# compix/Monte-Carlo-Raytracer

Measured on AMD Instinct MI355X. Metric: Mpaths/sec + achieved HBM GB/s, San-Miguel 1920x1080 at 1/2/4/8 MI355X, higher is better.
Workload: dtype f32; 1 GPU; san_miguel_proxy 1920x1080, unidirectional PT, maxDepth 2, random sampler, 1 spp per step, box-filter accumulate; width=1920, height=1080, triangles=9984786, max_depth=2, global_batch=1, bvh=RadeonRays-identical SAH, device build, parallelism=tile-split 8-row bands x 1 + 1 RCCL band gather, frames_per_launch=32, max_frames_per_call=32

## Files before the change

### include/mcrt_capi.h

```cpp
#ifndef MCRT_CAPI_H
#define MCRT_CAPI_H

#include <stddef.h>
#include <stdint.h>

#ifdef __cplusplus
extern "C" {
#endif

#define MCRT_API __attribute__((visibility("default")))

typedef int mcrt_status;
#define MCRT_OK                   0
#define MCRT_ERROR_INVALID_ARG    1
#define MCRT_ERROR_OUT_OF_MEMORY  2
#define MCRT_ERROR_DEVICE         3
#define MCRT_ERROR_NOT_READY      4
#define MCRT_ERROR_NO_DEVICE      5

typedef struct __attribute__((aligned(16))) { float x, y, z, w; } mcrt_float4;
typedef mcrt_float4 mcrt_float3;
typedef struct __attribute__((aligned(8))) { float x, y; } mcrt_float2;
typedef struct __attribute__((aligned(16))) { mcrt_float4 m0, m1, m2, m3; } mcrt_mat4;

// ... 164 lines not shown
MCRT_API mcrt_status mcrt_ctx_gather_chase_compact(mcrt_ctx ctx, uint64_t records, double leaf_frac, int steps,
                                                   int iters, double* gsteps);

MCRT_API mcrt_status mcrt_scene_create(mcrt_ctx ctx, const mcrt_scene_desc* desc, mcrt_scene* out);
MCRT_API mcrt_status mcrt_scene_destroy(mcrt_scene scene);
MCRT_API mcrt_status mcrt_scene_update_lights(mcrt_scene scene, const mcrt_light* lights, uint32_t n);
MCRT_API mcrt_status mcrt_scene_update_materials(mcrt_scene scene, const mcrt_material* m, uint32_t n);
MCRT_API mcrt_status mcrt_scene_update_shapes(mcrt_scene scene, const mcrt_shape* s, uint32_t n);
MCRT_API mcrt_status mcrt_scene_update_vertices(mcrt_scene scene, uint32_t first, uint32_t count,
                                                const mcrt_float4* positions, const mcrt_float4* normals);
MCRT_API mcrt_status mcrt_scene_update_vertices_device(mcrt_scene scene, uint32_t first, uint32_t count,
                                                       const void* d_positions, const void* d_normals);
MCRT_API mcrt_status mcrt_accel_build(mcrt_scene scene, const mcrt_accel_opts* opts);
MCRT_API mcrt_status mcrt_accel_update_transforms(mcrt_scene scene, const mcrt_shape* shapes, uint32_t n,
                                                  const mcrt_mat4* world_to_local );
MCRT_API mcrt_status mcrt_accel_refit(mcrt_scene scene);
MCRT_API mcrt_status mcrt_accel_update_info(mcrt_scene scene, int32_t* path, double* ms);
MCRT_API mcrt_status mcrt_accel_info(mcrt_scene scene, uint64_t* num_nodes, uint64_t* device_bytes,
                                     double* build_ms, uint32_t* num_triangles);
MCRT_API mcrt_status mcrt_accel_layout(mcrt_scene scene, int32_t* two_level, uint32_t* num_meshes,
                                       uint32_t* num_instances, int32_t* depth);
MCRT_API mcrt_status mcrt_accel_read_records(mcrt_scene scene, float* out, uint64_t max_records,
                                             uint64_t* num_records);
typedef struct mcrt_obj_scene_s* mcrt_obj_scene;
#define MCRT_OBJ_MIPS            1
#define MCRT_OBJ_EMISSIVE_LIGHTS 2
MCRT_API mcrt_status mcrt_obj_load(const char* path, uint32_t flags, mcrt_obj_scene* out);
MCRT_API mcrt_status mcrt_obj_add_directional_light(mcrt_obj_scene s, const float dir[3], const float intensity[3]);
MCRT_API mcrt_status mcrt_obj_add_point_light(mcrt_obj_scene s, const float pos[3], const float intensity[3]);
MCRT_API mcrt_status mcrt_obj_scene_desc(mcrt_obj_scene s, mcrt_scene_desc* desc);
MCRT_API const char* mcrt_obj_warnings(mcrt_obj_scene s);
MCRT_API void mcrt_obj_free(mcrt_obj_scene s);

MCRT_API mcrt_status mcrt_accel_builder(mcrt_scene scene, int32_t* builder);
MCRT_API mcrt_status mcrt_accel_build_host_records(const mcrt_scene_desc* desc, const mcrt_accel_opts* opts,
                                                   float* out_records, uint64_t max_records,
                                                   uint64_t* num_records, int32_t* info);

MCRT_API mcrt_status mcrt_accel_refit_host_records(const mcrt_scene_desc* desc, const mcrt_accel_opts* opts,
                                                   const mcrt_shape* moved_shapes,
                                                   const mcrt_mat4* moved_world_to_local,
                                                   float* out_records, uint64_t max_records,
                                                   uint64_t* num_records, int32_t* info);

MCRT_API mcrt_status mcrt_trace_closest(mcrt_scene scene, const mcrt_ray* d_rays, int32_t n,
                                        mcrt_intersection* d_hits);
// ... 176 lines not shown
```

### monte-carlo-raytracer_amd/csrc/mcrt_accel.cpp

```cpp
#include <hip/hip_runtime.h>

#include <algorithm>
#include <cassert>
#include <chrono>
#include <cstdio>
#include <cstdlib>
#include <cstring>
#include <string>
#include <vector>

#include "mcrt_host.h"

using mcrt::fail, mcrt::env_int;
using Clock = std::chrono::steady_clock;

static double ms_since(Clock::time_point t0) {
    return std::chrono::duration<double, std::milli>(Clock::now() - t0).count();
}

bool mcrt::accel_ready(mcrt_scene s) { return (bool)s->accel.dNodes; }
const float4* mcrt::accel_nodes(mcrt_scene s) { return s->accel.dNodes.get(); }
int mcrt::accel_spill_cap(mcrt_scene s) { return s->accel.spillCap; }
const float* mcrt::accel_world_box(mcrt_scene s) { return s->accel.tree.box; }

// ... 95 lines not shown
    a.refitParent.reset();
    a.refitArrive.reset();
    a.refitQOff.reset();
    a.refitFlag.reset();
    a.tree = mcrt::TreeInfo();
    a.qRoot = 0;
    a.packets = false;
}

static mcrt_status finish(mcrt_scene s, bool boxFromRoot) {
    mcrt_ctx ctx = s->ctx;
    AccelState& a = s->accel;
    mcrt::TreeInfo& t = a.tree;
    a.packets = !t.twoLevel && 2 * t.depth <= MCRT_PK_STACK && t.numNodes < (1u << 26) &&
                env_int("MCRT_CAMERA_PACKETS", 1) != 0;
    if (!a.dScratch) HIPCHK(ctx, a.dScratch.alloc(256));
    HIPCHK(ctx, hipMemset(a.dScratch.get(), 0, 256 * sizeof(int)));
    if (!t.twoLevel) {
        mcrt::launch_leaf_parents(a.dNodes.get(), (uint32_t)t.numNodes, ctx->stream);
        HIPCHK(ctx, hipStreamSynchronize(ctx->stream));
    }
    if (!t.twoLevel && env_int("MCRT_QUANT_NODES", 1) != 0) {
        DevBuf<float4> q;
        const hipError_t e = mcrt::build_qnodes(a.dNodes.get(), (uint32_t)t.numNodes, q, ctx->stream);
        if (e == hipSuccess) {
            a.dQNodes = std::move(q);
        } else if (e != hipErrorNotSupported && e != hipErrorOutOfMemory) {
            return fail(ctx, MCRT_ERROR_DEVICE, std::string("compact records: ") + hipGetErrorString(e));
        } else {
            (void)hipGetLastError();
        }
    }
    apply_spill_cap(a);
    if (boxFromRoot) {
        float root[16];
        HIPCHK(ctx, hipMemcpy(root, a.dNodes.get(), sizeof(root), hipMemcpyDeviceToHost));
        mcrt::root_record_box(root, t.box);
    }
    a.qRoot = !t.twoLevel && t.numNodes == 1 ? 1u : 0u;
    return MCRT_OK;
}

static mcrt_status commit(mcrt_scene s, const mcrt_accel_opts* opts, DevBuf<float4>& nodes, const mcrt::TreeInfo& info,
                          mcrt::HostTree* host, Clock::time_point t0) {
    AccelState& a = s->accel;
    drop(a);
    a.dNodes = std::move(nodes);
// ... 157 lines not shown
    HIPCHK(ctx, hipStreamSynchronize(ctx->stream));
    HIPCHK(ctx, hipDeviceSynchronize());
    if (a.tree.twoLevel) {
        mcrt_accel_opts o = a.lastOpts;
        const mcrt_status st = mcrt_accel_build(s, a.haveOpts ? &o : nullptr);
        if (st != MCRT_OK) return st;
        a.updatePath = 3;
        a.updateMs = ms_since(t0);
        return MCRT_OK;
    }
    hipStream_t st = ctx->stream;
    const uint32_t n = (uint32_t)a.tree.numNodes;
    [[maybe_unused]] const int depth0 = a.tree.depth, cap0 = a.spillCap;
    [[maybe_unused]] const bool packets0 = a.packets;
    if (!a.refitParent) {
        DevBuf<int> parent, arrive, flag;
        DevBuf<uint32_t> qoff;
        HIPCHK(ctx, parent.alloc(n));
        HIPCHK(ctx, arrive.alloc(n));
        HIPCHK(ctx, flag.alloc(4));
        HIPCHK(ctx, mcrt::launch_refit_parents(a.dNodes.get(), n, parent.get(), st));
        if (a.dQNodes) {
            size_t total = 0;
            HIPCHK(ctx, mcrt::refit_qnode_offsets(a.dNodes.get(), n, qoff, &total, st));
            if (total != a.dQNodes.size()) return fail(ctx, MCRT_ERROR_DEVICE, "compact records: size changed without a build");
        }
        a.refitParent = std::move(parent);
        a.refitArrive = std::move(arrive);
        a.refitFlag = std::move(flag);
        a.refitQOff = std::move(qoff);
    }
    {
        Timed t(ctx, K_REFIT, nullptr, (int64_t)n);
        HIPCHK(ctx, mcrt::launch_refit(a.dNodes.get(), n, s->dShapes.get(), (uint32_t)s->shapes.size(), s->dIndices.get(),
                                       s->dPositions.get(), a.refitParent.get(), a.refitArrive.get(), st));
    }
    int unbounded = 0;
    if (a.dQNodes) {
        Timed t(ctx, K_REFIT_QNODES, nullptr, (int64_t)n);
        HIPCHK(ctx, mcrt::refit_qnodes(a.dNodes.get(), n, a.refitQOff.get(), a.dQNodes.get(), a.refitFlag.get(), st));
    }
    float root[16];
    if (a.dQNodes) HIPCHK(ctx, hipMemcpyAsync(&unbounded, a.refitFlag.get(), sizeof(int), hipMemcpyDeviceToHost, st));
    HIPCHK(ctx, hipMemcpyAsync(root, a.dNodes.get(), sizeof(root), hipMemcpyDeviceToHost, st));
    HIPCHK(ctx, hipStreamSynchronize(st));
    if (unbounded) {
        a.dQNodes.reset();
// ... 29 lines not shown
    if (!s) return fail(nullptr, MCRT_ERROR_INVALID_ARG, "scene is NULL");
    const AccelState& a = s->accel;
    if (!a.dNodes) return fail(s->ctx, MCRT_ERROR_NOT_READY, "mcrt_accel_build has not been called");
    if (two_level) *two_level = a.tree.twoLevel ? 1 : 0;
    if (num_meshes) *num_meshes = (uint32_t)a.tree.numMeshes;
    if (num_instances) *num_instances = (uint32_t)a.tree.numInstances;
    if (depth) *depth = a.tree.depth;
    return MCRT_OK;
}

MCRT_API mcrt_status mcrt_accel_read_records(mcrt_scene s, float* out, uint64_t max_records, uint64_t* num_records) {
    if (!s || !num_records) return fail(s ? s->ctx : nullptr, MCRT_ERROR_INVALID_ARG, "NULL argument");
    const AccelState& a = s->accel;
    if (!a.dNodes) return fail(s->ctx, MCRT_ERROR_INVALID_ARG, "scene has no acceleration structure");
    *num_records = a.tree.numNodes;
    if (!out) return MCRT_OK;
    mcrt_ctx ctx = s->ctx;
    hipSetDevice(ctx->device);
    HIPCHK(ctx, hipStreamSynchronize(ctx->stream));
    HIPCHK(ctx, hipMemcpy(out, a.dNodes.get(), 64 * std::min<uint64_t>(max_records, a.tree.numNodes), hipMemcpyDeviceToHost));
    return MCRT_OK;
}

MCRT_API mcrt_status mcrt_accel_builder(mcrt_scene s, int32_t* builder) {
    if (!s || !builder) return fail(s ? s->ctx : nullptr, MCRT_ERROR_INVALID_ARG, "NULL argument");
    *builder = s->accel.tree.builder;
    return MCRT_OK;
}

}
```

### monte-carlo-raytracer_amd/csrc/mcrt_host.h

```cpp
#pragma once
#include <climits>
#include <cstddef>
#include <string>
#include <vector>

#include "mcrt_devbuf.h"
#include "mcrt_internal.h"

using mcrt::DevBuf;

#define MCRT_ATROUS_MAX_LEVELS 8

enum KernelId {
    K_PRIMARY, K_SHADE0, K_SHADEN, K_SHADOW, K_EXTEND, K_ACCUM, K_TRACE_CLOSEST, K_TRACE_ANY,
    K_BDPT_START, K_BDPT_VERTEX, K_BDPT_CONNECT, K_BDPT_VIS, K_BDPT_GATHER, K_SHADOW_EXTEND,
    K_GUIDES, K_MOMENTS, K_ATROUS_PREP,
    K_ATROUS,
    K_TEMPORAL = K_ATROUS + MCRT_ATROUS_MAX_LEVELS, K_TEMPORAL_VAR, K_GUIDES_MOTION, K_TEMPORAL_MOTION,
    K_TILE_ERROR, K_TILE_LIST,
    K_REFIT, K_REFIT_QNODES,
    K_COUNT
};

struct mcrt_ctx_s {
// ... 2 lines not shown
    hipStream_t stream = nullptr;
    int numCUs = 256;
    bool profiling = false;
    bool countHints = false;
    int* dFlags = nullptr;
    std::string error;
    struct Pending {
        int kernel;
        hipEvent_t a, b;
        const int* countDev;
        const int* countDev2;
        int64_t items;
    };
    std::vector<Pending> pending;
    double totalMs[K_COUNT] = {};
    int64_t launches[K_COUNT] = {};
    int64_t items[K_COUNT] = {};
};

struct AccelState {
    DevBuf<float4> dNodes;
    mcrt::TreeInfo tree;
    DevBuf<float4> dQNodes;
    uint32_t qRoot = 0;
    bool packets = false;
    double buildMs = 0.0;
    DevBuf<uint32_t> dSpill;
    int spillCap = 0;
    DevBuf<int> dScratch;
    DevBuf<uint32_t> dHintCell;
    int hintBits = 0;
    bool hintAllocFailed = false;
    mcrt_accel_opts lastOpts = {};
    bool haveOpts = false;
    mcrt::Bvh2lTop top2l;
    mcrt::TopBuildDev* topDev = nullptr;
    int updatePath = 0;
    double updateMs = 0.0;
    DevBuf<int> refitParent;
    DevBuf<int> refitArrive;
    DevBuf<uint32_t> refitQOff;
    DevBuf<int> refitFlag;
    ~AccelState() { mcrt::top_build_destroy(topDev); }
};

struct mcrt_scene_s {
// ... 254 lines not shown
```

### monte-carlo-raytracer_amd/csrc/mcrt_internal.h

```cpp
#pragma once
#include <hip/hip_runtime.h>
#include <stdint.h>
#include <cstddef>
#include <string>

#include "../../include/mcrt_capi.h"

struct SceneArgs {
    const mcrt_shape* shapes;
    const uint32_t* indices;
    const float4* positions;
    const float2* uvs;
    const float4* normals;
    const mcrt_texture_desc* textures;
    const uint8_t* texData;
    const uint32_t* sobol;
    const mcrt_light* lights;
    const mcrt_material* materials;
    const float4* nodes;
    const float4* surf;
    const uint32_t* surfBase;
    int numLights;
};

// ... 118 lines not shown
void launch_shade0(const SceneArgs& s, const FrameArgs& f, const mcrt_camera* cam, const float4* hits,
                   float4* radiance, const QueueArgs& q, hipStream_t st, int tileSlots = -1);
void launch_shadeN(const SceneArgs& s, const FrameArgs& f, int bounce, const int* countIn, const float4* qO,
                   const float4* qD, const float4* qT, const float4* hits, float4* radiance, const QueueArgs& q,
                   int maxCount, hipStream_t st);
void launch_aov(const SceneArgs& s, const FrameArgs& f, const mcrt_camera* cam, const float4* hits, int which,
                float4* out, hipStream_t st);
void launch_guides(const SceneArgs& s, const FrameArgs& f, const mcrt_camera* cam, const float4* hits,
                   float4* normalPlane, float4* albedoDepth, hipStream_t st);
void launch_pose_snapshot(const mcrt_shape* shapes, PrevPose* out, int n, hipStream_t st);
void launch_guides_motion(const SceneArgs& s, const FrameArgs& f, const mcrt_camera* cam, const float4* hits,
                          float4* normalPlane, float4* albedoDepth, const PrevPose* prev, float4* motion,
                          float4* prevNormal, hipStream_t st);
void launch_moments(const FrameArgs& f, int frame, const float4* radiance, float2* moments, hipStream_t st,
                    const uint32_t* list = nullptr, int listLen = 0, const uint32_t* tileCount = nullptr);
void launch_accumulate(const FrameArgs& f, int frame, const mcrt_filter* filters, int filterStride, const float4* radiance, float4* wsum, float* wts,
                       float4* image, hipStream_t st, const uint32_t* list = nullptr, int listLen = 0,
                       const uint32_t* tileCount = nullptr);
void launch_tonemap(int n, float Lwhite, const float4* in, float4* out, hipStream_t st);
void launch_leaf_parents(float4* nodes, uint32_t n, hipStream_t st);
void launch_tile_order(const uint32_t* cost, int n, uint32_t* order, hipStream_t st);
template <class T>
class DevBuf;
hipError_t build_qnodes(const float4* nodes, uint32_t n, DevBuf<float4>& q, hipStream_t st);
hipError_t qnode_offsets(uint32_t* units, uint32_t* off, uint32_t n, size_t* total, hipStream_t st);
hipError_t refit_qnode_offsets(const float4* nodes, uint32_t n, DevBuf<uint32_t>& off, size_t* total, hipStream_t st);
hipError_t refit_qnodes(const float4* nodes, uint32_t n, const uint32_t* off, float4* q, int* flag, hipStream_t st);
hipError_t launch_refit_parents(const float4* nodes, uint32_t n, int* parent, hipStream_t st);
hipError_t launch_refit(float4* nodes, uint32_t n, const mcrt_shape* dShapes, uint32_t numShapes, const uint32_t* dIndices,
                        const float4* dPositions, const int* parent, int* arrive, hipStream_t st);
void launch_bdpt_start(const SceneArgs& s, const FrameArgs& f, const BdptArgs& b, const mcrt_camera* cam,
                       const BdptQueue& camQ, const BdptQueue& lightQ, hipStream_t st);
void launch_bdpt_vertex(const SceneArgs& s, const FrameArgs& f, const BdptArgs& b, int depth, const BdptQueue& qIn,
                        const float4* hits, const BdptQueue& qOut, int maxCount, hipStream_t st);
void launch_bdpt_connect(const SceneArgs& s, const FrameArgs& f, const BdptArgs& b, const mcrt_camera* cam,
                         const BdptQueue& q, hipStream_t st);
constexpr int BDPT_VIS_MAX_WAVES = 65536;
void launch_bdpt_vis(const TraceCtx& c, const BdptArgs& b, const BdptQueue& q, int maxCount, hipStream_t st);
void launch_bdpt_gather(const FrameArgs& f, const BdptArgs& b, float4* radiance, const float* chunk,
                        size_t chunkPixels, hipStream_t st);
void launch_bdpt_splat_pack(const FrameArgs& f, size_t chunkPixels, const float4* splat, float* out, hipStream_t st);
void launch_bdpt_clear_splat(int n, float4* splat, hipStream_t st);
void launch_splat_hist(const BdptArgs& b, int* hist, hipStream_t st);
struct SplatOffsets { int off[64]; };
void launch_splat_group(const BdptArgs& b, SplatOffsets off, int* cursor, float4* dst, hipStream_t st);
void launch_splat_unpack(const float4* recv, int n, float4* splat, hipStream_t st);
}

#include <vector>
// ... 118 lines not shown
```

### monte-carlo-raytracer_amd/csrc/mcrt_qnodes.hip

```cpp
#include <rocprim/device/device_scan.hpp>

#include "mcrt_devbuf.h"
#include "mcrt_device.h"
#include "mcrt_internal.h"
#include "mcrt_traverse.h"

using mcrt::DevBuf;

__global__ __launch_bounds__(256) void k_leaf_parents(float4* __restrict__ nodes, uint32_t n) {
    const uint32_t i = blockIdx.x * 256 + threadIdx.x;
    if (i >= n) return;
    const int4 w = *reinterpret_cast<const int4*>(&nodes[4 * (size_t)i + 3]);
    if (w.x < 0) return;
    const int ch[2] = {w.x, w.y};
    for (int k = 0; k < 2; ++k) {
        if ((uint32_t)ch[k] >= n) continue;
        int* cw = reinterpret_cast<int*>(&nodes[4 * (size_t)ch[k] + 3]);
        if (cw[0] == -1) cw[1] = (int)i;
    }
}

__global__ __launch_bounds__(256) void k_qnodes_sizes(const float4* __restrict__ nodes, uint32_t n,
                                                      uint32_t* __restrict__ units, int* __restrict__ notDfs) {
    const uint32_t i = blockIdx.x * 256 + threadIdx.x;
    if (i >= n) return;
    const int4 w = *reinterpret_cast<const int4*>(&nodes[4 * (size_t)i + 3]);
    units[i] = w.x >= 0 ? 2u : 3u;
    if (w.x >= 0 && w.x != (int)i + 1) atomicOr(notDfs, 1);
}

MCRT_DEV bool quantExp(float lo0, float hi0, float lo1, float hi1, float& o, uint32_t& e) {
    o = fminf(lo0, lo1);
    const float ext = fmaxf(hi0, hi1) - o;
    if (!(ext >= 0.0f) || ext == __builtin_inff()) return false;
    int k = -126;
    if (ext > 0.0f) frexpf(ext * (1.0f / 250.0f), &k);
    e = (uint32_t)min(max(k + 127, 1), 254);
    return true;
}
MCRT_DEV bool quantBytes(float lo0, float hi0, float lo1, float hi1, float o, float sc, uint32_t& bytes) {
    const float b[4] = {lo0, hi0, lo1, hi1};
    bytes = 0;
    for (int j = 0; j < 4; ++j) {
        const bool up = (j & 1) != 0;
        int q = (int)(up ? ceilf((b[j] - o) / sc) : floorf((b[j] - o) / sc));
        q = min(max(q, 0), 255);
        if (up) {
            while (q < 255 && fmaf((float)q, sc, o) < b[j]) ++q;
            if (fmaf((float)q, sc, o) < b[j]) return false;
        } else {
            while (q > 0 && fmaf((float)q, sc, o) > b[j]) --q;
            if (fmaf((float)q, sc, o) > b[j]) return false;
        }
        bytes |= (uint32_t)q << (8 * j);
    }
    return true;
}

__global__ __launch_bounds__(256) void k_qnodes_convert(const float4* __restrict__ nodes, uint32_t n,
                                                        const uint32_t* __restrict__ off, float4* __restrict__ q,
                                                        int* __restrict__ fail) {
    const uint32_t i = blockIdx.x * 256 + threadIdx.x;
    if (i >= n) return;
    const float4 n0 = nodes[4 * (size_t)i], n1 = nodes[4 * (size_t)i + 1], n2 = nodes[4 * (size_t)i + 2];
    const int4 w = *reinterpret_cast<const int4*>(&nodes[4 * (size_t)i + 3]);
    float4* dst = q + off[i];
    if (w.x >= 0) {
        float ox, oy, oz;
        uint32_t bx = 0, by = 0, bz = 0, ex = 0, ey = 0, ez = 0;
        bool ok = quantExp(n0.x, n0.y, n1.x, n1.y, ox, ex) && quantExp(n0.z, n0.w, n1.z, n1.w, oy, ey) &&
                  quantExp(n2.x, n2.y, n2.z, n2.w, oz, ez) && (uint32_t)w.y < n;
        const uint32_t leaf0 = ok && reinterpret_cast<const int4*>(&nodes[4 * (size_t)w.x + 3])->x < 0 ? 1u : 0u;
        const uint32_t leaf1 = ok && reinterpret_cast<const int4*>(&nodes[4 * (size_t)w.y + 3])->x < 0 ? 1u : 0u;
        uint32_t meta = ex | (ey << 9) | (ez << 18) | (leaf0 << 27);
        if (ok && ey > 1 && quantBytes(n0.z, n0.w, n1.z, n1.w, oy, qScales(meta - (1u << 9)).y, by)) meta -= 1u << 9;
        if (ok && ez > 1 && quantBytes(n2.x, n2.y, n2.z, n2.w, oz, qScales(meta - (1u << 18)).z, bz)) meta -= 1u << 18;
        const QScales sc = qScales(meta);
        ok = ok && quantBytes(n0.x, n0.y, n1.x, n1.y, ox, sc.x, bx) && quantBytes(n0.z, n0.w, n1.z, n1.w, oy, sc.y, by) &&
             quantBytes(n2.x, n2.y, n2.z, n2.w, oz, sc.z, bz);
        if (!ok) {
            atomicOr(fail, 1);
            return;
        }
        dst[0] = make_float4(ox, oy, oz, __uint_as_float((off[w.y] << 1) | leaf1));
        dst[1] = make_float4(__uint_as_float(bx), __uint_as_float(by), __uint_as_float(bz), __uint_as_float(meta));
        return;
    }
    bool slow = true;
    const int par = w.y;
    if (par >= 0 && (uint32_t)par < n) {
        const float4 p0 = nodes[4 * (size_t)par], p1 = nodes[4 * (size_t)par + 1], p2 = nodes[4 * (size_t)par + 2];
        const bool right = reinterpret_cast<const int4*>(&nodes[4 * (size_t)par + 3])->y == (int)i;
        const f3 lo = right ? f3{p1.x, p1.z, p2.z} : f3{p0.x, p0.z, p2.x};
        const f3 hi = right ? f3{p1.y, p1.w, p2.w} : f3{p0.y, p0.w, p2.y};
        const f3 v0 = ld3(n0), v1 = v0 + ld3(n1), v2 = v0 + ld3(n2);
        const f3 l = f3{fminf(fminf(v0.x, v1.x), v2.x), fminf(fminf(v0.y, v1.y), v2.y), fminf(fminf(v0.z, v1.z), v2.z)};
        const f3 h = f3{fmaxf(fmaxf(v0.x, v1.x), v2.x), fmaxf(fmaxf(v0.y, v1.y), v2.y), fmaxf(fmaxf(v0.z, v1.z), v2.z)};
        slow = __float_as_uint(l.x) != __float_as_uint(lo.x) || __float_as_uint(l.y) != __float_as_uint(lo.y) ||
               __float_as_uint(l.z) != __float_as_uint(lo.z) || __float_as_uint(h.x) != __float_as_uint(hi.x) ||
               __float_as_uint(h.y) != __float_as_uint(hi.y) || __float_as_uint(h.z) != __float_as_uint(hi.z);
    }
    dst[0] = n0;
    dst[1] = n1;
    dst[2] = make_float4(n2.x, n2.y, n2.z, __uint_as_float(i | (slow ? 0x80000000u : 0u)));
}

namespace mcrt {

void launch_leaf_parents(float4* nodes, uint32_t n, hipStream_t st) {
    if (n == 0) return;
    hipLaunchKernelGGL(k_leaf_parents, dim3((n + 255) / 256), dim3(256), 0, st, nodes, n);
}

hipError_t qnode_offsets(uint32_t* units, uint32_t* off, uint32_t n, size_t* total, hipStream_t st) {
    *total = 0;
    if (n == 0 || n >= (1u << 30)) return hipErrorNotSupported;
    DevBuf<uint8_t> tmp;
    size_t tmpBytes = 0;
    uint32_t last[2] = {0, 0};
    hipError_t e = rocprim::exclusive_scan(nullptr, tmpBytes, units, off, 0u, (size_t)n, rocprim::plus<uint32_t>(), st);
    if (e == hipSuccess) e = (hipError_t)tmp.alloc(tmpBytes);
    if (e == hipSuccess) e = rocprim::exclusive_scan(tmp.get(), tmpBytes, units, off, 0u, (size_t)n, rocprim::plus<uint32_t>(), st);
    if (e == hipSuccess) e = hipMemcpyAsync(&last[0], off + n - 1, 4, hipMemcpyDeviceToHost, st);
    if (e == hipSuccess) e = hipMemcpyAsync(&last[1], units + n - 1, 4, hipMemcpyDeviceToHost, st);
    if (e == hipSuccess) e = hipStreamSynchronize(st);
    if (e != hipSuccess) return e;
    *total = (size_t)last[0] + last[1];
    return *total >= ((size_t)1 << 31) ? hipErrorNotSupported : hipSuccess;
}

hipError_t build_qnodes(const float4* nodes, uint32_t n, DevBuf<float4>& q, hipStream_t st) {
    q.reset();
    if (n == 0) return hipErrorNotSupported;
    DevBuf<uint32_t> units, off;
    DevBuf<int> flags;
    int h[2] = {0, 0};
    size_t total = 0;
    hipError_t e = (hipError_t)units.alloc(n);
    if (e == hipSuccess) e = (hipError_t)off.alloc(n);
    if (e == hipSuccess) e = (hipError_t)flags.alloc(2);
    if (e == hipSuccess) e = hipMemsetAsync(flags.get(), 0, 2 * sizeof(int), st);
    if (e != hipSuccess) return e;
    hipLaunchKernelGGL(k_qnodes_sizes, dim3((n + 255) / 256), dim3(256), 0, st, nodes, n, units.get(), flags.get());
    e = hipMemcpyAsync(h, flags.get(), sizeof(int), hipMemcpyDeviceToHost, st);
    if (e == hipSuccess) e = qnode_offsets(units.get(), off.get(), n, &total, st);
    if (e == hipSuccess && h[0] != 0) e = hipErrorNotSupported;
    if (e == hipSuccess) e = (hipError_t)q.alloc(total);
    if (e == hipSuccess) {
        hipLaunchKernelGGL(k_qnodes_convert, dim3((n + 255) / 256), dim3(256), 0, st, nodes, n, off.get(), q.get(),
                           flags.get() + 1);
        e = hipMemcpyAsync(h + 1, flags.get() + 1, sizeof(int), hipMemcpyDeviceToHost, st);
    }
    if (e == hipSuccess) e = hipStreamSynchronize(st);
    if (e == hipSuccess && h[1] != 0) e = hipErrorNotSupported;
    if (e != hipSuccess) q.reset();
    return e;
}

hipError_t refit_qnode_offsets(const float4* nodes, uint32_t n, DevBuf<uint32_t>& off, size_t* total, hipStream_t st) {
    off.reset();
    *total = 0;
    if (n == 0) return hipErrorNotSupported;
    DevBuf<uint32_t> units;
    DevBuf<int> flag;
    hipError_t e = (hipError_t)units.alloc(n);
    if (e == hipSuccess) e = (hipError_t)off.alloc(n);
    if (e == hipSuccess) e = (hipError_t)flag.alloc(1);
    if (e == hipSuccess) e = hipMemsetAsync(flag.get(), 0, sizeof(int), st);
    if (e == hipSuccess) {
        hipLaunchKernelGGL(k_qnodes_sizes, dim3((n + 255) / 256), dim3(256), 0, st, nodes, n, units.get(), flag.get());
        e = qnode_offsets(units.get(), off.get(), n, total, st);
    }
    if (e != hipSuccess) off.reset();
    return e;
}

hipError_t refit_qnodes(const float4* nodes, uint32_t n, const uint32_t* off, float4* q, int* flag, hipStream_t st) {
    const hipError_t e = hipMemsetAsync(flag, 0, sizeof(int), st);
    if (e != hipSuccess) return e;
    hipLaunchKernelGGL(k_qnodes_convert, dim3((n + 255) / 256), dim3(256), 0, st, nodes, n, off, q, flag);
    return hipGetLastError();
}

}
```

### monte-carlo-raytracer_amd/csrc/mcrt_traverse.h

```cpp
#pragma once
#include "mcrt_device.h"
#include "mcrt_internal.h"

#define STACK_LDS 16

#define LAY_PLAIN 0
#define LAY_QUANT 1
#define LAY_TWO_LEVEL 3
template <typename K>
inline K pickLayout(const TraceCtx& c, K twoLevel, K plain) {
    return c.twoLevel ? twoLevel : plain;
}
template <typename K>
inline K pickLayout(const TraceCtx& c, K twoLevel, K quant, K plain) {
    return c.twoLevel ? twoLevel : c.qnodes ? quant : plain;
}

MCRT_DEV uint32_t waveClockNow() { return (uint32_t)__builtin_amdgcn_s_memrealtime(); }
MCRT_DEV void waveClockStore(uint32_t* clk, uint32_t t0) {
    if (clk && (threadIdx.x & 63) == 0) {
        clk[2 * blockIdx.x] = t0;
        clk[2 * blockIdx.x + 1] = waveClockNow();
    }
}
// ... 407 lines not shown
                constexpr bool SX = (O & 1) != 0, SY = (O & 2) != 0, SZ = (O & 4) != 0;
                const float axn = fmaf(SX ? hi0.x : lo0.x, inv.x, oxi.x), axf = fmaf(SX ? lo0.x : hi0.x, inv.x, oxi.x);
                const float ayn = fmaf(SY ? hi0.y : lo0.y, inv.y, oxi.y), ayf = fmaf(SY ? lo0.y : hi0.y, inv.y, oxi.y);
                const float azn = fmaf(SZ ? hi0.z : lo0.z, inv.z, oxi.z), azf = fmaf(SZ ? lo0.z : hi0.z, inv.z, oxi.z);
                const float bxn = fmaf(SX ? hi1.x : lo1.x, inv.x, oxi.x), bxf = fmaf(SX ? lo1.x : hi1.x, inv.x, oxi.x);
                const float byn = fmaf(SY ? hi1.y : lo1.y, inv.y, oxi.y), byf = fmaf(SY ? lo1.y : hi1.y, inv.y, oxi.y);
                const float bzn = fmaf(SZ ? hi1.z : lo1.z, inv.z, oxi.z), bzf = fmaf(SZ ? lo1.z : hi1.z, inv.z, oxi.z);
                a0 = fmaxf(fmaxf(axn, ayn), fmaxf(azn, 0.0f));
                a1 = minFar(axf, ayf, azf, tc);
                b0 = fmaxf(fmaxf(bxn, byn), fmaxf(bzn, 0.0f));
                b1 = minFar(bxf, byf, bzf, tc);
            } else {
                const float ax0 = fmaf(lo0.x, inv.x, oxi.x), ax1 = fmaf(hi0.x, inv.x, oxi.x);
                const float ay0 = fmaf(lo0.y, inv.y, oxi.y), ay1 = fmaf(hi0.y, inv.y, oxi.y);
                const float az0 = fmaf(lo0.z, inv.z, oxi.z), az1 = fmaf(hi0.z, inv.z, oxi.z);
                const float bx0 = fmaf(lo1.x, inv.x, oxi.x), bx1 = fmaf(hi1.x, inv.x, oxi.x);
                const float by0 = fmaf(lo1.y, inv.y, oxi.y), by1 = fmaf(hi1.y, inv.y, oxi.y);
                const float bz0 = fmaf(lo1.z, inv.z, oxi.z), bz1 = fmaf(hi1.z, inv.z, oxi.z);
                a0 = fmaxf(fmaxf(fmaxf(fminf(ax0, ax1), fminf(ay0, ay1)), fminf(az0, az1)), 0.0f);
                a1 = minFar(fmaxf(ax0, ax1), fmaxf(ay0, ay1), fmaxf(az0, az1), tc);
                b0 = fmaxf(fmaxf(fmaxf(fminf(bx0, bx1), fminf(by0, by1)), fminf(bz0, bz1)), 0.0f);
                b1 = minFar(fmaxf(bx0, bx1), fmaxf(by0, by1), fmaxf(bz0, bz1), tc);
            }
            const uint32_t cl = ref + 4u + ((b.w >> 27) & 1u);
            const uint32_t cr = __float_as_uint(a.w);
            const bool h0 = a0 <= a1, h1 = b0 <= b1;
            const bool c1first = h1 && (a0 > b0);
            if (h0 && h1) {
                if (sp == STACK_LDS) {
                    if (spillTop + STACK_LDS - 1 <= c.spillCap) {
                        for (int k = 1; k < STACK_LDS; ++k) spill[(size_t)(spillTop + k - 1) * 64] = stk[k * 64];
                        spillTop += STACK_LDS - 1;
                    } else {
                        *c.overflow = 1;
                    }
                    sp = 1;
                }
                stk[sp * 64] = c1first ? cl : cr;
                ++sp;
            }
            next = (h0 || h1) ? ((c1first || !h0) ? cr : cl) : POP;
        } else {
            next = POP;
            const uint32_t w = __float_as_uint(e2.w);
            const float4 e1 = make_float4(__uint_as_float(b.x), __uint_as_float(b.y), __uint_as_float(b.z), 0.0f);
            const float th = r.mask != __float_as_int(a.w) ? triRaw(r, a, e1, e2) : __builtin_inff();
            if (th <= tc) {
                bool boxHit;
// ... 321 lines not shown
```

### monte-carlo-raytracer_amd/mcrt/lib.py

```python
import ctypes
import weakref
import os

import numpy as np

from . import PKG_DIR
from . import types as T

_DEFAULT_LIB = os.path.join(os.path.dirname(PKG_DIR), "libmcrt.so")
LIB_PATH = os.environ.get("MCRT_LIB_PATH") or _DEFAULT_LIB
HEADER = os.path.join(os.path.dirname(os.path.dirname(PKG_DIR)), "include", "mcrt_capi.h")

_c = ctypes
_vp = _c.c_void_p
_lib = None

SIGNATURES = {
    "mcrt_version": (_c.c_char_p, []),
    "mcrt_last_error": (_c.c_char_p, [_vp]),
    "mcrt_ctx_create": (_c.c_int, [_c.c_int, _c.POINTER(_vp)]),
    "mcrt_ctx_destroy": (_c.c_int, [_vp]),
    "mcrt_ctx_synchronize": (_c.c_int, [_vp]),
    "mcrt_ctx_set_stream": (_c.c_int, [_vp, _vp]),
    "mcrt_ctx_set_profiling": (_c.c_int, [_vp, _c.c_int]),
# ... 13 lines not shown
    "mcrt_scene_update_vertices_device": (_c.c_int, [_vp, _c.c_uint32, _c.c_uint32, _vp, _vp]),
    "mcrt_accel_refit": (_c.c_int, [_vp]),
    "mcrt_accel_build": (_c.c_int, [_vp, _vp]),
    "mcrt_accel_update_transforms": (_c.c_int, [_vp, _vp, _c.c_uint32, _vp]),
    "mcrt_accel_update_info": (_c.c_int, [_vp, _c.POINTER(_c.c_int32), _c.POINTER(_c.c_double)]),
    "mcrt_accel_refit_host_records": (_c.c_int, [_vp, _vp, _vp, _vp, _vp, _c.c_uint64, _c.POINTER(_c.c_uint64), _vp]),
    "mcrt_accel_info": (_c.c_int, [_vp, _vp, _vp, _vp, _vp]),
    "mcrt_accel_layout": (_c.c_int, [_vp, _vp, _vp, _vp, _vp]),
    "mcrt_accel_builder": (_c.c_int, [_vp, _vp]),
    "mcrt_bdpt_splats_copy": (_c.c_int, [_vp, _vp]),
    "mcrt_bdpt_splat_layout": (_c.c_int, [_vp, _c.POINTER(_c.c_uint64), _c.POINTER(_c.c_int32)]),
    "mcrt_framebuffer_stream": (_c.c_int, [_vp, _c.POINTER(_vp)]),
    "mcrt_bdpt_gather": (_c.c_int, [_vp, _vp]),
    "mcrt_framebuffer_set_splat_exchange": (_c.c_int, [_vp, _c.c_int32]),
    "mcrt_bdpt_splats_sparse": (_c.c_int, [_vp, _vp, _c.c_int64, _c.POINTER(_c.c_int64), _c.c_int32]),
    "mcrt_bdpt_gather_sparse": (_c.c_int, [_vp, _vp, _c.c_int64]),
    "mcrt_obj_load": (_c.c_int, [_c.c_char_p, _c.c_uint32, _vp]),
    "mcrt_obj_add_directional_light": (_c.c_int, [_vp, _vp, _vp]),
    "mcrt_obj_add_point_light": (_c.c_int, [_vp, _vp, _vp]),
    "mcrt_obj_scene_desc": (_c.c_int, [_vp, _vp]),
    "mcrt_obj_warnings": (_c.c_char_p, [_vp]),
    "mcrt_obj_free": (None, [_vp]),
    "mcrt_accel_read_records": (_c.c_int, [_vp, _vp, _c.c_uint64, _vp]),
    "mcrt_accel_build_host_records": (_c.c_int, [_vp, _vp, _vp, _c.c_uint64, _c.POINTER(_c.c_uint64), _vp]),
    "mcrt_trace_closest": (_c.c_int, [_vp, _vp, _c.c_int32, _vp]),
    "mcrt_trace_any": (_c.c_int, [_vp, _vp, _c.c_int32, _vp]),
    "mcrt_trace_closest_count": (_c.c_int, [_vp, _vp, _vp, _c.c_int32, _vp, _vp, _c.POINTER(_vp)]),
    "mcrt_trace_any_count": (_c.c_int, [_vp, _vp, _vp, _c.c_int32, _vp, _vp, _c.POINTER(_vp)]),
    "mcrt_event_wait": (_c.c_int, [_vp]),
    "mcrt_event_destroy": (_c.c_int, [_vp]),
    "mcrt_framebuffer_create": (_c.c_int, [_vp, _c.c_uint32, _c.c_uint32, _c.POINTER(_vp)]),
    "mcrt_framebuffer_destroy": (_c.c_int, [_vp]),
    "mcrt_framebuffer_set_frames_in_flight": (_c.c_int, [_vp, _c.c_int32]),
    "mcrt_render_frame": (_c.c_int, [_vp, _vp, _vp, _vp]),
    "mcrt_accumulate": (_c.c_int, [_vp, _vp, _c.c_int32]),
    "mcrt_render_frames": (_c.c_int, [_vp, _vp, _vp, _c.c_int32, _vp]),
    "mcrt_accumulate_frames": (_c.c_int, [_vp, _vp, _c.c_int32, _c.c_int32]),
    "mcrt_framebuffer_device_ptrs": (_c.c_int, [_vp, _vp, _vp, _vp, _vp]),
    "mcrt_framebuffer_read": (_c.c_int, [_vp, _c.c_int, _vp]),
    "mcrt_framebuffer_read_frame": (_c.c_int, [_vp, _c.c_int32, _vp]),
    "mcrt_framebuffer_stats": (_c.c_int, [_vp, _vp, _vp, _vp]),
    "mcrt_framebuffer_copy_device": (_c.c_int, [_vp, _c.c_int, _vp]),
    "mcrt_framebuffer_copy_device_frame": (_c.c_int, [_vp, _c.c_int32, _vp]),
    "mcrt_framebuffer_set_accumulation": (_c.c_int, [_vp, _vp, _vp]),
    "mcrt_framebuffer_bands_pack": (_c.c_int, [_vp, _vp]),
    "mcrt_framebuffer_bands_unpack": (_c.c_int, [_vp, _vp, _c.c_int32]),
# ... 159 lines not shown
def event_wait(ev):
    _check(lib().mcrt_event_wait(ev))


def event_destroy(ev):
    _check(lib().mcrt_event_destroy(ev))


def build_host_records(scene, **opts):
    desc = scene.desc()
    w2l = opts.get("world_to_local")
    if w2l is not None:
        opts["world_to_local"] = np.ascontiguousarray(w2l, np.float32)
    o = accel_opts(**opts)
    n = _c.c_uint64()
    _check(lib().mcrt_accel_build_host_records(_c.byref(desc), _c.byref(o), None, 0, _c.byref(n), None))
    rec = np.zeros((n.value, 16), np.float32)
    info = np.zeros(4, np.int32)
    _check(lib().mcrt_accel_build_host_records(_c.byref(desc), _c.byref(o), _p(rec), n.value, _c.byref(n), _p(info)))
    return rec, {"two_level": int(info[0]), "top_records": int(info[1]), "depth": int(info[2]),
                 "meshes": int(info[3])}


def refit_host_records(scene, moved_shapes, world_to_local=None, **opts):
    desc = scene.desc()
    o = accel_opts(**opts)
    moved = np.ascontiguousarray(moved_shapes)
    w2l = None if world_to_local is None else np.ascontiguousarray(world_to_local, np.float32)
    n = _c.c_uint64()
    f = lib().mcrt_accel_refit_host_records
    _check(f(_c.byref(desc), _c.byref(o), _p(moved), _p(w2l), None, 0, _c.byref(n), None))
    rec = np.zeros((n.value, 16), np.float32)
    info = np.zeros(4, np.int32)
    _check(f(_c.byref(desc), _c.byref(o), _p(moved), _p(w2l), _p(rec), n.value, _c.byref(n), _p(info)))
    return rec, {"two_level": int(info[0]), "top_records": int(info[1]), "depth": int(info[2]),
                 "meshes": int(info[3])}


class DeviceScene:
    def __init__(self, ctx, scene, build=True, cost=10.0, bins=64, sah=True, device_build=False,
                 force_2level=False, force_flat=False, world_to_local=None):
        self.ctx = ctx
        self.scene = scene
        self._desc = scene.desc()
        h = _vp()
        _check(lib().mcrt_scene_create(ctx.h, _c.byref(self._desc), _c.byref(h)), ctx.h)
        self.h = h
        ctx._adopt(self)
        if build:
            self.build(cost, bins, sah, device_build, force_2level, force_flat, world_to_local)

    def build(self, cost=10.0, bins=64, sah=True, device_build=False, force_2level=False, force_flat=False,
              world_to_local=None):
        w2l = None if world_to_local is None else np.ascontiguousarray(world_to_local, np.float32)
        opts = accel_opts(cost, bins, sah, device_build, force_2level, force_flat, w2l)
        _check(lib().mcrt_accel_build(self.h, _c.byref(opts)), self.ctx.h)

    def layout(self):
        tl, nm, ni, dp = _c.c_int32(), _c.c_uint32(), _c.c_uint32(), _c.c_int32()
        _check(lib().mcrt_accel_layout(self.h, _c.byref(tl), _c.byref(nm), _c.byref(ni), _c.byref(dp)), self.ctx.h)
        return {"two_level": tl.value, "meshes": nm.value, "instances": ni.value, "depth": dp.value}

    def records(self):
        n = _c.c_uint64()
        _check(lib().mcrt_accel_read_records(self.h, None, 0, _c.byref(n)), self.ctx.h)
        rec = np.zeros((n.value, 16), np.float32)
        _check(lib().mcrt_accel_read_records(self.h, _p(rec), n.value, _c.byref(n)), self.ctx.h)
        return rec

    def builder(self):
        b = _c.c_int32()
        _check(lib().mcrt_accel_builder(self.h, _c.byref(b)), self.ctx.h)
        return b.value

    def info(self):
        nn, nb, ms, nt = _c.c_uint64(), _c.c_uint64(), _c.c_double(), _c.c_uint32()
        _check(lib().mcrt_accel_info(self.h, _c.byref(nn), _c.byref(nb), _c.byref(ms), _c.byref(nt)), self.ctx.h)
        return {"nodes": nn.value, "bytes": nb.value, "build_ms": ms.value, "triangles": nt.value}

    def update_lights(self, lights):
        self._lights = np.ascontiguousarray(lights)
        _check(lib().mcrt_scene_update_lights(self.h, _p(self._lights), len(self._lights)), self.ctx.h)

    def update_materials(self, mats):
        self._mats = np.ascontiguousarray(mats)
        _check(lib().mcrt_scene_update_materials(self.h, _p(self._mats), len(self._mats)), self.ctx.h)

    def update_shapes(self, shapes):
        self._shapes = np.ascontiguousarray(shapes)
        _check(lib().mcrt_scene_update_shapes(self.h, _p(self._shapes), len(self._shapes)), self.ctx.h)

# ... 399 lines not shown
```

Measured before the change: 1936 Mpaths/s.

## Reorder compact BVH nodes into cache-line-aligned treelets for traversal locality

Replaces the depth-first prefix-sum placement of quantized BVH nodes with a host-computed ordering. By default each parent is packed together with its two children inside one 128-byte (8-unit) block, and blocks are padded so they never straddle the boundary. Child references become a left offset plus a step field, so traversal can fetch both siblings from nearby memory. This is meant to cut cache misses and HBM traffic during traversal, in exchange for padding overhead and a host round trip during build and refit. It also adds API entry points to read back the compact layout.

Result: faster. 1974 Mpaths/s, median of 6 (+2.0%).

```diff
diff --git a/include/mcrt_capi.h b/include/mcrt_capi.h
--- a/include/mcrt_capi.h
+++ b/include/mcrt_capi.h
@@ -210,6 +210,10 @@
                                        uint32_t* num_instances, int32_t* depth);
 MCRT_API mcrt_status mcrt_accel_read_records(mcrt_scene scene, float* out, uint64_t max_records,
                                              uint64_t* num_records);
+MCRT_API mcrt_status mcrt_accel_read_compact(mcrt_scene scene, void* out, uint64_t max_units, uint64_t* num_units,
+                                             uint32_t* root_ref);
+MCRT_API mcrt_status mcrt_accel_compact_order(const int32_t* kids, uint32_t n, int32_t order, uint32_t* off,
+                                              uint64_t* num_units);
 typedef struct mcrt_obj_scene_s* mcrt_obj_scene;
 #define MCRT_OBJ_MIPS            1
 #define MCRT_OBJ_EMISSIVE_LIGHTS 2
diff --git a/monte-carlo-raytracer_amd/csrc/mcrt_accel.cpp b/monte-carlo-raytracer_amd/csrc/mcrt_accel.cpp
--- a/monte-carlo-raytracer_amd/csrc/mcrt_accel.cpp
+++ b/monte-carlo-raytracer_amd/csrc/mcrt_accel.cpp
@@ -141,7 +141,9 @@
     }
     if (!t.twoLevel && env_int("MCRT_QUANT_NODES", 1) != 0) {
         DevBuf<float4> q;
-        const hipError_t e = mcrt::build_qnodes(a.dNodes.get(), (uint32_t)t.numNodes, q, ctx->stream);
+        const int order = env_int("MCRT_QNODE_ORDER", mcrt::QORDER_TREELETS);
+        a.qOrder = order == mcrt::QORDER_SIBLINGS ? order : mcrt::QORDER_TREELETS;
+        const hipError_t e = mcrt::build_qnodes(a.dNodes.get(), (uint32_t)t.numNodes, a.qOrder, q, ctx->stream);
         if (e == hipSuccess) {
             a.dQNodes = std::move(q);
         } else if (e != hipErrorNotSupported && e != hipErrorOutOfMemory) {
@@ -345,7 +347,7 @@
         HIPCHK(ctx, mcrt::launch_refit_parents(a.dNodes.get(), n, parent.get(), st));
         if (a.dQNodes) {
             size_t total = 0;
-            HIPCHK(ctx, mcrt::refit_qnode_offsets(a.dNodes.get(), n, qoff, &total, st));
+            HIPCHK(ctx, mcrt::refit_qnode_offsets(a.dNodes.get(), n, a.qOrder, qoff, &total, st));
             if (total != a.dQNodes.size()) return fail(ctx, MCRT_ERROR_DEVICE, "compact records: size changed without a build");
         }
         a.refitParent = std::move(parent);
@@ -421,6 +423,35 @@
     return MCRT_OK;
 }
 
+MCRT_API mcrt_status mcrt_accel_read_compact(mcrt_scene s, void* out, uint64_t max_units, uint64_t* num_units,
+                                             uint32_t* root_ref) {
+    if (!s || !num_units) return fail(s ? s->ctx : nullptr, MCRT_ERROR_INVALID_ARG, "NULL argument");
+    const AccelState& a = s->accel;
+    if (!a.dNodes) return fail(s->ctx, MCRT_ERROR_INVALID_ARG, "scene has no acceleration structure");
+    *num_units = a.dQNodes.size();
+    if (root_ref) *root_ref = a.qRoot;
+    if (!out || !a.dQNodes) return MCRT_OK;
+    mcrt_ctx ctx = s->ctx;
+    hipSetDevice(ctx->device);
+    HIPCHK(ctx, hipStreamSynchronize(ctx->stream));
+    HIPCHK(ctx, hipMemcpy(out, a.dQNodes.get(), 16 * std::min<uint64_t>(max_units, a.dQNodes.size()), hipMemcpyDeviceToHost));
+    return MCRT_OK;
+}
+
+MCRT_API mcrt_status mcrt_accel_compact_order(const int32_t* kids, uint32_t n, int32_t order, uint32_t* off,
+                                              uint64_t* num_units) {
+    if (!kids || !off || !num_units || n == 0 || order < 1 || order > 2)
+        return fail(nullptr, MCRT_ERROR_INVALID_ARG, "NULL argument, no records or an unknown order");
+    for (uint32_t i = 0; i < n; ++i) {
+        const int32_t l = kids[2 * (size_t)i], r = kids[2 * (size_t)i + 1];
+        if (l < 0) continue;
+        if ((uint32_t)l <= i || (uint32_t)l >= n || (uint32_t)r <= i || (uint32_t)r >= n || l == r)
+            return fail(nullptr, MCRT_ERROR_INVALID_ARG, "child indices must lie above their parent's");
+    }
+    *num_units = mcrt::qnode_order_offsets(kids, n, order, off);
+    return MCRT_OK;
+}
+
 MCRT_API mcrt_status mcrt_accel_builder(mcrt_scene s, int32_t* builder) {
     if (!s || !builder) return fail(s ? s->ctx : nullptr, MCRT_ERROR_INVALID_ARG, "NULL argument");
     *builder = s->accel.tree.builder;
diff --git a/monte-carlo-raytracer_amd/csrc/mcrt_host.h b/monte-carlo-raytracer_amd/csrc/mcrt_host.h
--- a/monte-carlo-raytracer_amd/csrc/mcrt_host.h
+++ b/monte-carlo-raytracer_amd/csrc/mcrt_host.h
@@ -48,6 +48,7 @@
     DevBuf<float4> dNodes;
     mcrt::TreeInfo tree;
     DevBuf<float4> dQNodes;
+    int qOrder = 0;
     uint32_t qRoot = 0;
     bool packets = false;
     double buildMs = 0.0;
diff --git a/monte-carlo-raytracer_amd/csrc/mcrt_internal.h b/monte-carlo-raytracer_amd/csrc/mcrt_internal.h
--- a/monte-carlo-raytracer_amd/csrc/mcrt_internal.h
+++ b/monte-carlo-raytracer_amd/csrc/mcrt_internal.h
@@ -164,9 +164,12 @@
 void launch_tile_order(const uint32_t* cost, int n, uint32_t* order, hipStream_t st);
 template <class T>
 class DevBuf;
-hipError_t build_qnodes(const float4* nodes, uint32_t n, DevBuf<float4>& q, hipStream_t st);
+enum { QORDER_SIBLINGS = 1, QORDER_TREELETS = 2 };
+hipError_t build_qnodes(const float4* nodes, uint32_t n, int order, DevBuf<float4>& q, hipStream_t st);
+size_t qnode_order_offsets(const int* kids, uint32_t n, int order, uint32_t* off);
 hipError_t qnode_offsets(uint32_t* units, uint32_t* off, uint32_t n, size_t* total, hipStream_t st);
-hipError_t refit_qnode_offsets(const float4* nodes, uint32_t n, DevBuf<uint32_t>& off, size_t* total, hipStream_t st);
+hipError_t refit_qnode_offsets(const float4* nodes, uint32_t n, int order, DevBuf<uint32_t>& off, size_t* total,
+                               hipStream_t st);
 hipError_t refit_qnodes(const float4* nodes, uint32_t n, const uint32_t* off, float4* q, int* flag, hipStream_t st);
 hipError_t launch_refit_parents(const float4* nodes, uint32_t n, int* parent, hipStream_t st);
 hipError_t launch_refit(float4* nodes, uint32_t n, const mcrt_shape* dShapes, uint32_t numShapes, const uint32_t* dIndices,
diff --git a/monte-carlo-raytracer_amd/csrc/mcrt_qnodes.hip b/monte-carlo-raytracer_amd/csrc/mcrt_qnodes.hip
--- a/monte-carlo-raytracer_amd/csrc/mcrt_qnodes.hip
+++ b/monte-carlo-raytracer_amd/csrc/mcrt_qnodes.hip
@@ -1,4 +1,6 @@
 #include <rocprim/device/device_scan.hpp>
+
+#include <vector>
 
 #include "mcrt_devbuf.h"
 #include "mcrt_device.h"
@@ -20,13 +22,13 @@
     }
 }
 
-__global__ __launch_bounds__(256) void k_qnodes_sizes(const float4* __restrict__ nodes, uint32_t n,
-                                                      uint32_t* __restrict__ units, int* __restrict__ notDfs) {
+__global__ __launch_bounds__(256) void k_qnodes_kids(const float4* __restrict__ nodes, uint32_t n,
+                                                     int2* __restrict__ kids, int* __restrict__ notDfs) {
     const uint32_t i = blockIdx.x * 256 + threadIdx.x;
     if (i >= n) return;
     const int4 w = *reinterpret_cast<const int4*>(&nodes[4 * (size_t)i + 3]);
-    units[i] = w.x >= 0 ? 2u : 3u;
-    if (w.x >= 0 && w.x != (int)i + 1) atomicOr(notDfs, 1);
+    kids[i] = w.x >= 0 ? make_int2(w.x, w.y) : make_int2(-1, -1);
+    if (w.x >= 0 && (w.x != (int)i + 1 || (uint32_t)w.y >= n || w.y <= w.x)) atomicOr(notDfs, 1);
 }
 
 MCRT_DEV bool quantExp(float lo0, float hi0, float lo1, float hi1, float& o, uint32_t& e) {
@@ -72,7 +74,8 @@
                   quantExp(n2.x, n2.y, n2.z, n2.w, oz, ez) && (uint32_t)w.y < n;
         const uint32_t leaf0 = ok && reinterpret_cast<const int4*>(&nodes[4 * (size_t)w.x + 3])->x < 0 ? 1u : 0u;
         const uint32_t leaf1 = ok && reinterpret_cast<const int4*>(&nodes[4 * (size_t)w.y + 3])->x < 0 ? 1u : 0u;
-        uint32_t meta = ex | (ey << 9) | (ez << 18) | (leaf0 << 27);
+        const uint32_t step = ok ? 2u * (off[w.y] - off[w.x]) + leaf1 - leaf0 : 0u;
+        uint32_t meta = ex | (ey << 9) | (ez << 18) | (step << 27);
         if (ok && ey > 1 && quantBytes(n0.z, n0.w, n1.z, n1.w, oy, qScales(meta - (1u << 9)).y, by)) meta -= 1u << 9;
         if (ok && ez > 1 && quantBytes(n2.x, n2.y, n2.z, n2.w, oz, qScales(meta - (1u << 18)).z, bz)) meta -= 1u << 18;
         const QScales sc = qScales(meta);
@@ -82,7 +85,7 @@
             atomicOr(fail, 1);
             return;
         }
-        dst[0] = make_float4(ox, oy, oz, __uint_as_float((off[w.y] << 1) | leaf1));
+        dst[0] = make_float4(ox, oy, oz, __uint_as_float((off[w.x] << 1) | leaf0));
         dst[1] = make_float4(__uint_as_float(bx), __uint_as_float(by), __uint_as_float(bz), __uint_as_float(meta));
         return;
     }
@@ -129,50 +132,95 @@
     return *total >= ((size_t)1 << 31) ? hipErrorNotSupported : hipSuccess;
 }
 
-hipError_t build_qnodes(const float4* nodes, uint32_t n, DevBuf<float4>& q, hipStream_t st) {
+size_t qnode_order_offsets(const int* kids, uint32_t n, int order, uint32_t* off) {
+    auto leaf = [&](uint32_t i) { return kids[2 * (size_t)i] < 0; };
+    auto units = [&](uint32_t i) { return leaf(i) ? 3u : 2u; };
+    auto fit = [](size_t cur, uint32_t u) { return (cur & 7u) + u > 8u ? (cur + 7u) & ~(size_t)7u : cur; };
+    size_t cur = 0;
+    auto place = [&](uint32_t i) { off[i] = (uint32_t)cur; cur += units(i); };
+    place(0);
+    if (order == QORDER_SIBLINGS) {
+        for (uint32_t i = 0; i < n; ++i) {
+            if (leaf(i)) continue;
+            const uint32_t l = (uint32_t)kids[2 * (size_t)i], r = (uint32_t)kids[2 * (size_t)i + 1];
+            cur = fit(cur, units(l) + units(r));
+            place(l);
+            place(r);
+        }
+        return cur;
+    }
+    std::vector<uint8_t> inner(n, 0);
+    auto treelet = [&](uint32_t g) {
+        if (leaf(g)) { cur = fit(cur, 3u); place(g); return; }
+        const uint32_t l = (uint32_t)kids[2 * (size_t)g], r = (uint32_t)kids[2 * (size_t)g + 1];
+        cur = fit(cur, 2u + units(l) + units(r));
+        place(g);
+        place(l);
+        place(r);
+        inner[l] = inner[r] = 1;
+    };
+    cur = 0;
+    treelet(0);
+    for (uint32_t i = 1; i < n; ++i) {
+        if (!inner[i] || leaf(i)) continue;
+        treelet((uint32_t)kids[2 * (size_t)i]);
+        treelet((uint32_t)kids[2 * (size_t)i + 1]);
+    }
+    return cur;
+}
+
+static hipError_t order_offsets(const float4* nodes, uint32_t n, int order, DevBuf<uint32_t>& off, size_t* total,
+                                hipStream_t st) {
+    off.reset();
+    *total = 0;
+    if (n == 0 || n >= (1u << 30)) return hipErrorNotSupported;
+    DevBuf<int2> kids;
+    DevBuf<int> flag;
+    int notDfs = 0;
+    hipError_t e = (hipError_t)kids.alloc(n);
+    if (e == hipSuccess) e = (hipError_t)flag.alloc(1);
+    if (e == hipSuccess) e = hipMemsetAsync(flag.get(), 0, sizeof(int), st);
+    if (e != hipSuccess) return e;
+    std::vector<int> hk(2 * (size_t)n);
+    hipLaunchKernelGGL(k_qnodes_kids, dim3((n + 255) / 256), dim3(256), 0, st, nodes, n, kids.get(), flag.get());
+    e = hipMemcpyAsync(hk.data(), kids.get(), 2 * sizeof(int) * (size_t)n, hipMemcpyDeviceToHost, st);
+    if (e == hipSuccess) e = hipMemcpyAsync(&notDfs, flag.get(), sizeof(int), hipMemcpyDeviceToHost, st);
+    if (e == hipSuccess) e = hipStreamSynchronize(st);
+    if (e != hipSuccess) return e;
+    if (notDfs) return hipErrorNotSupported;
+    kids.reset();
+    std::vector<uint32_t> ho(n);
+    const size_t units = qnode_order_offsets(hk.data(), n, order, ho.data());
+    if (units >= ((size_t)1 << 31)) return hipErrorNotSupported;
+    e = (hipError_t)off.alloc(n);
+    if (e == hipSuccess) e = hipMemcpyAsync(off.get(), ho.data(), sizeof(uint32_t) * (size_t)n, hipMemcpyHostToDevice, st);
+    if (e == hipSuccess) e = hipStreamSynchronize(st);
+    if (e != hipSuccess) off.reset();
+    else *total = units;
+    return e;
+}
+
+hipError_t build_qnodes(const float4* nodes, uint32_t n, int order, DevBuf<float4>& q, hipStream_t st) {
     q.reset();
-    if (n == 0) return hipErrorNotSupported;
-    DevBuf<uint32_t> units, off;
-    DevBuf<int> flags;
-    int h[2] = {0, 0};
+    DevBuf<uint32_t> off;
+    DevBuf<int> flag;
+    int h = 0;
     size_t total = 0;
-    hipError_t e = (hipError_t)units.alloc(n);
-    if (e == hipSuccess) e = (hipError_t)off.alloc(n);
-    if (e == hipSuccess) e = (hipError_t)flags.alloc(2);
-    if (e == hipSuccess) e = hipMemsetAsync(flags.get(), 0, 2 * sizeof(int), st);
-    if (e != hipSuccess) return e;
-    hipLaunchKernelGGL(k_qnodes_sizes, dim3((n + 255) / 256), dim3(256), 0, st, nodes, n, units.get(), flags.get());
-    e = hipMemcpyAsync(h, flags.get(), sizeof(int), hipMemcpyDeviceToHost, st);
-    if (e == hipSuccess) e = qnode_offsets(units.get(), off.get(), n, &total, st);
-    if (e == hipSuccess && h[0] != 0) e = hipErrorNotSupported;
+    hipError_t e = order_offsets(nodes, n, order, off, &total, st);
+    if (e == hipSuccess) e = (hipError_t)flag.alloc(1);
     if (e == hipSuccess) e = (hipError_t)q.alloc(total);
-    if (e == hipSuccess) {
-        hipLaunchKernelGGL(k_qnodes_convert, dim3((n + 255) / 256), dim3(256), 0, st, nodes, n, off.get(), q.get(),
-                           flags.get() + 1);
-        e = hipMemcpyAsync(h + 1, flags.get() + 1, sizeof(int), hipMemcpyDeviceToHost, st);
-    }
-    if (e == hipSuccess) e = hipStreamSynchronize(st);
-    if (e == hipSuccess && h[1] != 0) e = hipErrorNotSupported;
+    if (e == hipSuccess) e = hipMemsetAsync(q.get(), 0, 16 * total, st);
+    if (e == hipSuccess) e = refit_qnodes(nodes, n, off.get(), q.get(), flag.get(), st);
+    if (e == hipSuccess) e = hipMemcpyAsync(&h, flag.get(), sizeof(int), hipMemcpyDeviceToHost, st);
+    if (e == hipSuccess) e = hipStreamSynchronize(st);
+    if (e == hipSuccess && h != 0) e = hipErrorNotSupported;
     if (e != hipSuccess) q.reset();
     return e;
 }
 
-hipError_t refit_qnode_offsets(const float4* nodes, uint32_t n, DevBuf<uint32_t>& off, size_t* total, hipStream_t st) {
-    off.reset();
-    *total = 0;
-    if (n == 0) return hipErrorNotSupported;
-    DevBuf<uint32_t> units;
-    DevBuf<int> flag;
-    hipError_t e = (hipError_t)units.alloc(n);
-    if (e == hipSuccess) e = (hipError_t)off.alloc(n);
-    if (e == hipSuccess) e = (hipError_t)flag.alloc(1);
-    if (e == hipSuccess) e = hipMemsetAsync(flag.get(), 0, sizeof(int), st);
-    if (e == hipSuccess) {
-        hipLaunchKernelGGL(k_qnodes_sizes, dim3((n + 255) / 256), dim3(256), 0, st, nodes, n, units.get(), flag.get());
-        e = qnode_offsets(units.get(), off.get(), n, total, st);
-    }
-    if (e != hipSuccess) off.reset();
-    return e;
+hipError_t refit_qnode_offsets(const float4* nodes, uint32_t n, int order, DevBuf<uint32_t>& off, size_t* total,
+                               hipStream_t st) {
+    return order_offsets(nodes, n, order, off, total, st);
 }
 
 hipError_t refit_qnodes(const float4* nodes, uint32_t n, const uint32_t* off, float4* q, int* flag, hipStream_t st) {
diff --git a/monte-carlo-raytracer_amd/csrc/mcrt_traverse.h b/monte-carlo-raytracer_amd/csrc/mcrt_traverse.h
--- a/monte-carlo-raytracer_amd/csrc/mcrt_traverse.h
+++ b/monte-carlo-raytracer_amd/csrc/mcrt_traverse.h
@@ -453,8 +453,8 @@
                 b0 = fmaxf(fmaxf(fmaxf(fminf(bx0, bx1), fminf(by0, by1)), fminf(bz0, bz1)), 0.0f);
                 b1 = minFar(fmaxf(bx0, bx1), fmaxf(by0, by1), fmaxf(bz0, bz1), tc);
             }
-            const uint32_t cl = ref + 4u + ((b.w >> 27) & 1u);
-            const uint32_t cr = __float_as_uint(a.w);
+            const uint32_t cl = __float_as_uint(a.w);
+            const uint32_t cr = cl + (b.w >> 27);
             const bool h0 = a0 <= a1, h1 = b0 <= b1;
             const bool c1first = h1 && (a0 > b0);
             if (h0 && h1) {
diff --git a/monte-carlo-raytracer_amd/mcrt/lib.py b/monte-carlo-raytracer_amd/mcrt/lib.py
--- a/monte-carlo-raytracer_amd/mcrt/lib.py
+++ b/monte-carlo-raytracer_amd/mcrt/lib.py
@@ -59,6 +59,8 @@
     "mcrt_obj_warnings": (_c.c_char_p, [_vp]),
     "mcrt_obj_free": (None, [_vp]),
     "mcrt_accel_read_records": (_c.c_int, [_vp, _vp, _c.c_uint64, _vp]),
+    "mcrt_accel_read_compact": (_c.c_int, [_vp, _vp, _c.c_uint64, _vp, _vp]),
+    "mcrt_accel_compact_order": (_c.c_int, [_vp, _c.c_uint32, _c.c_int32, _vp, _vp]),
     "mcrt_accel_build_host_records": (_c.c_int, [_vp, _vp, _vp, _c.c_uint64, _c.POINTER(_c.c_uint64), _vp]),
     "mcrt_trace_closest": (_c.c_int, [_vp, _vp, _c.c_int32, _vp]),
     "mcrt_trace_any": (_c.c_int, [_vp, _vp, _c.c_int32, _vp]),
@@ -264,6 +266,14 @@
                  "meshes": int(info[3])}
 
 
+def compact_order(kids, order):
+    kids = np.ascontiguousarray(kids, np.int32)
+    off = np.zeros(len(kids), np.uint32)
+    n = _c.c_uint64()
+    _check(lib().mcrt_accel_compact_order(_p(kids), len(kids), order, _p(off), _c.byref(n)))
+    return off, n.value
+
+
 def refit_host_records(scene, moved_shapes, world_to_local=None, **opts):
     desc = scene.desc()
     o = accel_opts(**opts)
@@ -309,6 +319,13 @@
         rec = np.zeros((n.value, 16), np.float32)
         _check(lib().mcrt_accel_read_records(self.h, _p(rec), n.value, _c.byref(n)), self.ctx.h)
         return rec
+
+    def compact_records(self):
+        n, root = _c.c_uint64(), _c.c_uint32()
+        _check(lib().mcrt_accel_read_compact(self.h, None, 0, _c.byref(n), _c.byref(root)), self.ctx.h)
+        rec = np.zeros((n.value, 4), np.uint32)
+        _check(lib().mcrt_accel_read_compact(self.h, _p(rec), n.value, _c.byref(n), _c.byref(root)), self.ctx.h)
+        return rec, root.value
 
     def builder(self):
         b = _c.c_int32()
```
